# ziatdinovmax/pyroVED

Measured on AMD Instinct MI355X. Metric: images/sec (SVI step), higher is better.
Workload: dtype bf16; 1 GPU; C2 iVAE 28x28 invariances=['r','t'] latent_dim=2 bernoulli, batch 256 per GPU (global 256), bf16 MFMA operands for the hidden-layer contractions (fp32 accumulate; fp32 elsewhere); the guide (fc encoder, sample, split) runs in the decoder launch's prologue in fp32, SVI step = ELBO+grads+Adam; parallelism=dp1

## Files before the change

### pyroved_amd/csrc/pv_elementwise.hip

```cpp
#include "pv_common.h"
#include "pv_kernels.h"
#include "pv_wgrad_small.h"
#include "pv_side.h"
#include "pv_sdec_fused.h"


__device__ __forceinline__ float block_sum_256(float v, float* sm ) {
  v = pv_wave_sum(v);
  pv_lds_barrier();
  if ((threadIdx.x & 63) == 0) sm[threadIdx.x >> 6] = v;
  pv_lds_barrier();
  return (sm[0] + sm[1]) + (sm[2] + sm[3]);
}

__global__ __launch_bounds__(256) void pv_head_fwd_kernel(PvHead h) {
  __shared__ float sm[4];
  const int total = h.B * h.z_dim;
  float lp = 0.0f, lq = 0.0f;
  for (int e = threadIdx.x; e < total; e += 256) {
    const int b = e / h.z_dim, i = e % h.z_dim;
    const int ldh = h.ldh > 0 ? h.ldh : 2 * h.z_dim;
    const float mu = h.head[(int64_t)b * ldh + i];
    const float sp = h.head[(int64_t)b * ldh + h.z_dim + i];
    const float sig = h.scale_direct ? sp : pv_softplus(sp);
// ... 1032 lines not shown
  if (t < p.hb.z_dim)
    pv_head_bwd_elem(p.hb, b, t, [&](int c) { return sh_tp[c]; }, [&](int k) { return sh_dzc[k]; },
                     p.enc_n > 0 ? sh_dh : nullptr);
  if (p.K > 0 && t == 0) {
    const float b1 = p.beta_disc, lK = logf((float)K);
    const float* al = p.alpha + (int64_t)b * K;
    float dot = 0.0f;
    for (int k = 0; k < K; ++k) {
      const float da = -(sh_ll[k] - b1 * lK - b1 * logf(al[k]) - b1);
      dot += al[k] * da;
    }
    const int ldh = p.hb.ldh > 0 ? p.hb.ldh : 2 * p.hb.z_dim;
    for (int k = 0; k < K; ++k) {
      const float da = -(sh_ll[k] - b1 * lK - b1 * logf(al[k]) - b1);
      p.hb.dhead[(int64_t)b * ldh + 2 * p.hb.z_dim + k] = al[k] * (da - dot);
      if (p.enc_n > 0) sh_dh[2 * p.hb.z_dim + k] = al[k] * (da - dot);
    }
  }
  LB_STAMP(4);
  if (p.enc_n <= 0) return;
  pv_lds_barrier();
  const int ne = p.enc_n;
  int cur = 0;
  {
    const pv_layer hd = p.enc_head, ll_ = p.enc_l[ne - 1];
    const float* Wh = p.enc_params + hd.w_off;
    for (int k = t; k < ll_.out_dim; k += 256) {
      float v = 0.0f;
      if (chain && k == t) {
#pragma unroll
        for (int o = 0; o < 16; ++o) v += o < hd.out_dim ? sh_dh[o] * whd[o] : 0.0f;
        for (int o = 16; o < hd.out_dim; ++o) v += sh_dh[o] * Wh[(int64_t)o * hd.in_dim + k];
      } else {
        for (int o = 0; o < hd.out_dim; ++o) v += sh_dh[o] * Wh[(int64_t)o * hd.in_dim + k];
      }
      v *= pv_act_grad2((chain && k == t) ? pf_act1 : p.enc_act[ne - 1][(int64_t)b * ll_.out_dim + k], 0.0f, ll_.act);
      p.enc_dp[ne - 1][(int64_t)b * ll_.out_dim + k] = v;
      sh_e[cur][k] = v;
    }
    pv_lds_barrier();
  }
  LB_STAMP(5);
  for (int li = ne - 1; li > 0; --li) {
    const pv_layer l = p.enc_l[li], lp = p.enc_l[li - 1];
    const float* W = p.enc_params + l.w_off;
    const bool pre = li == ne - 1;
    const int k = ck, half = chalf;
    const int jh = l.out_dim >> 1, j0 = half * jh;
    float v = 0.0f;
    if (k < l.in_dim) {
      if (!pre) {
        const float* wc = W + k;
#pragma unroll
        for (int u = 0; u < 16; ++u)
#pragma unroll
          for (int i = 0; i < 4; ++i) wv4[u][i] = (4 * u + i < jh) ? wc[(int64_t)(j0 + 4 * u + i) * l.in_dim] : 0.0f;
      }
      f32x4 acc4 = {0.0f, 0.0f, 0.0f, 0.0f};
#pragma unroll
      for (int u = 0; u < 16; ++u)
        if (4 * u < jh) acc4 += *reinterpret_cast<const f32x4*>(&sh_e[cur][j0 + 4 * u]) * wv4[u];
      v = (acc4[0] + acc4[1]) + (acc4[2] + acc4[3]);
    }
    sh_p[half][k] = v;
    pv_lds_barrier();
    if (half == 0 && k < l.in_dim) {
      float y = sh_p[0][k] + sh_p[1][k];
      const float hv = pre ? pf_act0 : p.enc_act[li - 1][(int64_t)b * lp.out_dim + k];
      y *= pv_act_grad2(hv, 0.0f, lp.act);
      p.enc_dp[li - 1][(int64_t)b * lp.out_dim + k] = y;
      sh_e[cur ^ 1][k] = y;
    }
    pv_lds_barrier();
    cur ^= 1;
  }
  LB_STAMP(6);
}

__global__ __launch_bounds__(256) void pv_latent_bwd_kernel(PvLatentBwd p) { pv_latent_bwd_block(p, blockIdx.x); }

__global__ __launch_bounds__(256) void pv_latent_bwd_reduce_kernel(PvLatentBwd p, const float* __restrict__ part,
                                                                   int G_, float* __restrict__ Gr, PvFusedOffsets o,
                                                                   int cd, int fmt) {
  __shared__ f32x4 smr[4][64];
#ifndef LB_EXP
#define LB_EXP 0
#endif
  const int nred = pv_fused_reduce_blocks(fmt);
  if ((int)blockIdx.x < nred) { if (!(LB_EXP & 1)) pv_sdec_fused_reduce_block(part, G_, Gr, o, cd, 0, blockIdx.x, smr, fmt); }
  else if (!(LB_EXP & 2)) pv_latent_bwd_block(p, blockIdx.x - nred);
}

int pv_latent_bwd_reduce(const PvLatentBwd& p, const float* part, int grid, float* G, const PvFusedOffsets& o, int cd,
                         hipStream_t s, int fmt) {
  if (p.H > 512 || p.lat_in > 64 + (p.K > 0 ? p.K : 0) || p.hb.z_dim > 256 || p.K > 128) return PV_EINVAL;
  PV_LAUNCH_FORK(pv_latent_bwd_reduce_kernel, dim3(pv_fused_reduce_blocks(fmt) + p.hb.B), dim3(256), 0, s, p, part, grid, G, o, cd, fmt);
  PV_LAUNCH_CHECK();
  return 0;
}

__global__ __launch_bounds__(256) void pv_rec_wgrad_kernel(const float* __restrict__ part, int G_, float* __restrict__ Gr, PvFusedOffsets o,
                                                           int cd, int fmt, PvWgradSmall w, PvRecAdam ra, int rwx) {
  __shared__ f32x4 smr[4][64];
  __shared__ float wpart[WG_WAVES][16][17];
  __shared__ float wrpart[WG_WAVES][16];
  const int nred = pv_fused_reduce_blocks(fmt), id = (int)blockIdx.x;
  if (id < nred) { if (!(rwx & 1)) pv_sdec_fused_reduce_block(part, G_, Gr, o, cd, 0, id, smr, fmt, (rwx & 4) ? PvRecAdam{} : ra); return; }
  if (rwx & 2) return;
  pv_wgrad_small_block(w, id - nred, (int)gridDim.x - nred, wpart, wrpart);
}

int pv_rec_wgrad(const float* part, int grid, float* G, const PvFusedOffsets& o, int cd, int fmt, const PvGemm* gs, int n,
                 const PvAdamFuse* adam, const PvFinishArgs* fin, hipStream_t s, unsigned* tick) {
  PvWgradSmall w;
  int guests = 0;
  const int tiles = pv_wgrad_small_fill(w, gs, n, adam, fin, &guests);
  if (tiles < 0) return tiles;
  const int fin_blocks = (fin && fin->scalars) ? 1 : 0;
  if (tick && !fin_blocks) return PV_EINVAL;
  w.tick = tick;
  PvRecAdam ra{};
  if (adam) { ra.a = *adam; ra.on = 1; }
  static const int rwx = pv_exp_int("PV_RW_EXP", 0);
  hipLaunchKernelGGL(pv_rec_wgrad_kernel, dim3(pv_fused_reduce_blocks(fmt) + tiles + fin_blocks), dim3(256), 0, s, part, grid, G, o, cd,
                     fmt, w, ra, rwx);
  PV_LAUNCH_CHECK();
  return 0;
}

int pv_latent_bwd(const PvLatentBwd& p, hipStream_t s) {
  if (p.H > 512 || p.lat_in > 64 + (p.K > 0 ? p.K : 0) || p.hb.z_dim > 256 || p.K > 128) return PV_EINVAL;
  hipLaunchKernelGGL(pv_latent_bwd_kernel, dim3(p.hb.B), dim3(256), 0, s, p);
  PV_LAUNCH_CHECK();
  return 0;
}

__global__ void pv_adam_kernel(float* __restrict__ p, float* __restrict__ g, float* __restrict__ m,
                               float* __restrict__ v, int64_t n, float b1, float b2, float eps, float step_size,
                               float bc2_sqrt) {
  for (int64_t i = (int64_t)blockIdx.x * blockDim.x + threadIdx.x; i < n; i += (int64_t)gridDim.x * blockDim.x) {
    pv_adam_update(p, g, m, v, i, g[i], b1, b2, eps, step_size, bc2_sqrt);
  }
}

__global__ void pv_adam_hist_kernel(float* __restrict__ p, float* __restrict__ g, float* __restrict__ m,
                                    float* __restrict__ v, int64_t n, float b1, float b2, float eps, float step_size,
                                    float bc2_sqrt, const float* __restrict__ ssrc, float* __restrict__ sdst, int ns) {
  if (blockIdx.x == 0 && (int)threadIdx.x < ns) sdst[threadIdx.x] = ssrc[threadIdx.x];
  for (int64_t i = (int64_t)blockIdx.x * blockDim.x + threadIdx.x; i < n; i += (int64_t)gridDim.x * blockDim.x) {
    pv_adam_update(p, g, m, v, i, g[i], b1, b2, eps, step_size, bc2_sqrt);
  }
}

extern "C" int pv_adam_step_hist(float* params, float* grads, float* m, float* v, int64_t n, float lr, float beta1,
                                 float beta2, float eps, int32_t step, const float* scalars_src, float* scalars_dst,
                                 int32_t n_scalars, void* stream) {
  PV_RANGE("pv_adam_step_hist");
  if (step < 1 || n < 0 || n_scalars < 0 || n_scalars > 256 || (n_scalars > 0 && (!scalars_src || !scalars_dst)))
    return PV_EINVAL;
  const double bc1 = 1.0 - pow((double)beta1, (double)step);
  const double bc2 = 1.0 - pow((double)beta2, (double)step);
  int blocks = (int)((n + 255) / 256);
  if (blocks > 2048) blocks = 2048;
  if (blocks < 1) blocks = 1;
  hipLaunchKernelGGL(pv_adam_hist_kernel, dim3(blocks), dim3(256), 0, (hipStream_t)stream, params, grads, m, v, n, beta1,
                     beta2, eps, (float)((double)lr / bc1), (float)sqrt(bc2), scalars_src, scalars_dst, (int)n_scalars);
  PV_LAUNCH_CHECK();
  return 0;
}

extern "C" int pv_adam_step(float* params, float* grads, float* m, float* v, int64_t n, float lr, float beta1,
                            float beta2, float eps, int32_t step, void* stream) {
  PV_RANGE("pv_adam_step");
  if (n <= 0) return 0;
  if (step < 1) return PV_EINVAL;
  const double bc1 = 1.0 - pow((double)beta1, (double)step);
  const double bc2 = 1.0 - pow((double)beta2, (double)step);
  const float step_size = (float)((double)lr / bc1);
  const float bc2_sqrt = (float)sqrt(bc2);
  int blocks = (int)((n + 255) / 256);
  if (blocks > 2048) blocks = 2048;
  hipLaunchKernelGGL(pv_adam_kernel, dim3(blocks), dim3(256), 0, (hipStream_t)stream, params, grads, m, v, n, beta1,
                     beta2, eps, step_size, bc2_sqrt);
  PV_LAUNCH_CHECK();
  return 0;
}

__global__ void pv_lik_elem_kernel(const float* __restrict__ a, const float* __restrict__ x, int64_t M, int lik,
                                   int sigmoid_out, float sig, float* __restrict__ loc, float* __restrict__ llrow,
                                   float* __restrict__ dlda, const float* __restrict__ pw, int64_t per) {
  for (int64_t e = (int64_t)blockIdx.x * blockDim.x + threadIdx.x; e < M; e += (int64_t)gridDim.x * blockDim.x) {
    float ll, d, lv;
    pv_lik_one(a[e], x[e], lik, sigmoid_out, sig, ll, d, lv);
    if (pw) { const float w = pw[e % per]; ll *= w; d *= w; }
    if (loc) loc[e] = lv;
    if (llrow) llrow[e] = ll;
    if (dlda) dlda[e] = d;
  }
}

__global__ __launch_bounds__(256) void pv_lik_rows_kernel(const float* __restrict__ a, const float* __restrict__ x, int64_t per,
                                                          int lik, int sigmoid_out, float sig, float* __restrict__ loc,
                                                          float* __restrict__ dlda, float* __restrict__ llb,
                                                          const float* __restrict__ pw) {
  __shared__ float sm[4];
  const int64_t base = (int64_t)blockIdx.x * per;
// ... 134 lines not shown
```

### pyroved_amd/csrc/pv_particles.hip

```cpp
#include "pv_particles.h"
#include <cmath>

#define PX_THREADS 128
#define PX_MAX_Z 256
#define PX_MAX_LAT 256

template <class D> __device__ __forceinline__ int px_coord_cols(const D& d) {
  if (d.coord_dim == 1) return d.has_t ? 1 : 0;
  if (d.coord_dim == 2) return (d.has_r ? 1 : 0) + (d.has_t ? 2 : 0) + (d.has_s ? 1 : 0);
  return 0;
}

__global__ __launch_bounds__(PX_THREADS) void pv_particle_expand_kernel(PvParticleExpand e) {
  __shared__ float sm[16];
  __shared__ float sh_z[PX_MAX_Z];
  __shared__ float sh_in[PX_MAX_LAT];
  const int b = blockIdx.x, t = threadIdx.x, zd = e.z_dim;
  const int idx = px_coord_cols(e), L = zd - idx, lat_in = L + e.c_dim;
  const float inv_p = 1.0f / (float)e.P;
  float lp = 0.0f, lq = 0.0f;
  for (int p = 0; p < e.P; ++p) {
    const int64_t s = (int64_t)p * e.B + b;
    for (int i = t; i < zd; i += PX_THREADS) {
      const float mu = e.head[(int64_t)b * e.ldh + i];
// ... 100 lines not shown
        for (int n = t; n < p.N; n += 256) {
          a[0] += p.llrow[r0 + n];
          if (!p.fwd_only)
            for (int c = 0; c < 4; ++c) a[1 + c] += p.rowtp[(int64_t)c * p.M + r0 + n];
        }
        for (int c = 0; c < 5; ++c) {
          const float v = pv_block_sum(a[c], sm);
          if (t == 0) sh_a[c] = v;
        }
      }
      if (!p.fwd_only) {
        for (int j = t; j < p.H; j += 256) {
          const float* ph = p.part_hz + (s * p.kmax) * p.H + j;
          float v = 0.0f;
          for (int kk = 0; kk < p.kmax; ++kk) v += ph[(int64_t)kk * p.H];
          p.dhz[s * p.H + j] = v;
          sh_dhz[j] = v;
        }
        __syncthreads();
        if (t < n_content) {
          float v = 0.0f;
          for (int j = 0; j < p.H; ++j) v += sh_dhz[j] * p.Wz[(int64_t)j * p.lat_in + t];
          sh_dzc[t] = v;
        }
      }
    }
    __syncthreads();
    const float w = p.sw[s];
    if (t == 0) ll_acc += w * (p.ll_s ? p.ll_s[s] : sh_a[0]);
    if (!p.fwd_only && t < zd) {
      const float dz = pv_head_dz(p.hb, t, [&](int c) { return sh_a[1 + c]; }, [&](int k) { return sh_dzc[k]; });
      const int64_t e = s * zd + t;
      float g, ds;
      pv_head_bwd_math_kl(p.hb.kl_mode, dz, p.hb.z[e], p.hb.head[(int64_t)b * ldh + t], p.hb.z_scale[(int64_t)b * zd + t], p.hb.eps[e],
                          p.hb.head[(int64_t)b * ldh + zd + t], p.hb.beta * w, p.hb.scale_direct, g, ds);
      acc_g += g;
      acc_ds += ds;
    }
    __syncthreads();
  }
  if (t == 0) p.llb[b] = p.llb_add ? ll_acc + p.llb_add[b] : ll_acc;
  if (p.fwd_only) return;
  if (t < zd) {
    p.hb.dhead[(int64_t)b * ldh + t] = acc_g;
    p.hb.dhead[(int64_t)b * ldh + zd + t] = acc_ds;
    sh_dh[t] = acc_g;
    sh_dh[zd + t] = acc_ds;
  }
  if (p.enc_n <= 0) return;
  __syncthreads();
  const int ne = p.enc_n;
  int cur = 0;
  {
    const pv_layer hd = p.enc_head, l = p.enc_l[ne - 1];
    const float* Wh = p.enc_params + hd.w_off;
    for (int k = t; k < l.out_dim; k += 256) {
      float v = 0.0f;
      for (int o = 0; o < hd.out_dim; ++o) v += sh_dh[o] * Wh[(int64_t)o * hd.in_dim + k];
      v *= pv_act_grad2(p.enc_act[ne - 1][(int64_t)b * l.out_dim + k], 0.0f, l.act);
      p.enc_dp[ne - 1][(int64_t)b * l.out_dim + k] = v;
      sh_e[cur][k] = v;
    }
    __syncthreads();
  }
  for (int li = ne - 1; li > 0; --li) {
    const pv_layer l = p.enc_l[li], lp = p.enc_l[li - 1];
    const float* W = p.enc_params + l.w_off;
    for (int k = t; k < l.in_dim; k += 256) {
      float v = 0.0f;
      for (int j = 0; j < l.out_dim; ++j) v += sh_e[cur][j] * W[(int64_t)j * l.in_dim + k];
      v *= pv_act_grad2(p.enc_act[li - 1][(int64_t)b * lp.out_dim + k], 0.0f, lp.act);
      p.enc_dp[li - 1][(int64_t)b * lp.out_dim + k] = v;
      sh_e[cur ^ 1][k] = v;
    }
    __syncthreads();
    cur ^= 1;
  }
}

__global__ __launch_bounds__(256) void pv_particle_bwd_kernel(PvParticleBwd p) { pv_particle_bwd_block(p, blockIdx.x); }

__global__ __launch_bounds__(256) void pv_particle_bwd_reduce_kernel(PvParticleBwd p, const float* __restrict__ part, int G_,
                                                                     float* __restrict__ Gr, PvFusedOffsets o, int cd, int fmt) {
  __shared__ f32x4 smr[4][64];
  const int nred = pv_fused_reduce_blocks(fmt);
  if ((int)blockIdx.x < nred) pv_sdec_fused_reduce_block(part, G_, Gr, o, cd, 0, blockIdx.x, smr, fmt);
  else pv_particle_bwd_block(p, blockIdx.x - nred);
}

static int particle_bwd_check(const PvParticleBwd& p) {
  if (p.P < 1 || p.hb.B < 1 || p.hb.z_dim < 1 || p.hb.z_dim > PX_MAX_Z || !p.sw || !p.llb) return PV_EINVAL;
  if (p.llkb) {
    if (!p.fwd_only && (!p.dzc || (p.hb.coord_dim > 0 && !p.dtp))) return PV_EINVAL;
  } else {
    if (p.H > 512 || p.lat_in > PX_MAX_LAT || p.kmax < 1) return PV_EINVAL;
    if (!p.part_rs && !p.llrow) return PV_EINVAL;
    if (!p.fwd_only && (!p.part_hz || !p.dhz || !p.Wz || (!p.part_rs && !p.rowtp))) return PV_EINVAL;
  }
  if (p.enc_n > 0) {
    if (p.enc_head.out_dim != 2 * p.hb.z_dim) return PV_EINVAL;
    for (int i = 0; i < p.enc_n; ++i)
      if (p.enc_l[i].out_dim > 256) return PV_EINVAL;
  }
  return 0;
}

int pv_particle_bwd(const PvParticleBwd& p, hipStream_t s) {
  PV_TRY(particle_bwd_check(p));
  hipLaunchKernelGGL(pv_particle_bwd_kernel, dim3(p.hb.B), dim3(256), 0, s, p);
  PV_LAUNCH_CHECK();
  return 0;
}

int pv_particle_bwd_reduce(const PvParticleBwd& p, const float* part, int grid, float* G, const PvFusedOffsets& o, int cd,
                           hipStream_t s, int rec_fmt) {
  PV_TRY(particle_bwd_check(p));
  hipLaunchKernelGGL(pv_particle_bwd_reduce_kernel, dim3(pv_fused_reduce_blocks(rec_fmt) + p.hb.B), dim3(256), 0, s, p, part, grid, G, o,
                     cd, rec_fmt);
  PV_LAUNCH_CHECK();
  return 0;
}

__global__ __launch_bounds__(64) void pv_renyi_weights_kernel(PvRenyiWeights r) {
  __shared__ float sh_a[PV_RENYI_MAX_P], sh_lp[PV_RENYI_MAX_P], sh_lq[PV_RENYI_MAX_P];
  const int b = blockIdx.x, t = threadIdx.x, zd = r.z_dim;
  const float oma = 1.0f - r.alpha;
  for (int p = 0; p < r.P; ++p) {
    const int64_t s = (int64_t)p * r.B + b;
    float lp = 0.0f, lq = 0.0f;
    for (int i = t; i < zd; i += 64) {
      const float z = r.z[s * zd + i], e = r.eps[s * zd + i], sig = r.z_scale[(int64_t)b * zd + i];
      lq += -(e * e) / 2.0f - logf(sig) - LOG_SQRT_2PI;
      lp += -(z * z) / 2.0f - LOG_SQRT_2PI;
    }
    lp = r.beta * pv_wave_sum(lp);
    lq = r.beta * pv_wave_sum(lq);
    if (t == 0) {
      sh_lp[p] = lp;
      sh_lq[p] = lq;
      sh_a[p] = oma * (r.llkb[s] + (lp - lq));
    }
  }
  if (t != 0) return;
  float m = sh_a[0];
  for (int p = 1; p < r.P; ++p) m = fmaxf(m, sh_a[p]);
  float sum = 0.0f;
  for (int p = 0; p < r.P; ++p) sum += expf(sh_a[p] - m);
  const float inv = 1.0f / sum, lsum = logf(sum);
  float klp = 0.0f, klq = 0.0f, ent = 0.0f;
  for (int p = 0; p < r.P; ++p) {
    const int64_t s = (int64_t)p * r.B + b;
    const float d = sh_a[p] - m, w = expf(d) * inv;
    r.sw[s] = w;
    if (r.weights_out) r.weights_out[s] = w;
    klp += w * sh_lp[p];
    klq += w * sh_lq[p];
    ent -= w * (d - lsum);
  }
  r.kl_part[2 * b] = klp;
  r.kl_part[2 * b + 1] = klq;
  r.c[b] = (ent - logf((float)r.P)) / oma;
}

int pv_renyi_weights(const PvRenyiWeights& r, hipStream_t s) {
  if (r.B < 1 || r.P < 1 || r.P > PV_RENYI_MAX_P || r.z_dim < 1 || !std::isfinite(r.alpha) || r.alpha == 1.0f) return PV_EINVAL;
  if (!r.llkb || !r.z || !r.eps || !r.z_scale || !r.sw || !r.kl_part || !r.c) return PV_EINVAL;
  hipLaunchKernelGGL(pv_renyi_weights_kernel, dim3(r.B), dim3(64), 0, s, r);
// ... 4 lines not shown
```

### pyroved_amd/csrc/pv_sdec_fused.h

```cpp
#pragma once
#include "pv_common.h"

#define FD_H 128
#define FD_UNIT 16
#define FD_WAVES 8
#define FD_REC (2 * FD_H * FD_H + 14 * FD_H)
#define PV_RS_W 8
#define FB_WIMG_BYTES (4 * FD_H * FD_H * 2 + 256)

struct PvFused {
  const float* x;
  const float* grid;
  const float* tp;
  const float* hz;
  float hz_scale;
  const float *Wc, *bc;
  const float *W1, *b1;
  const float *W2, *b2;
  const float *wo, *bo;
  float* llrow;
  float* loc;
  float* rowtp;
  float* part_hz;
  float* part_rs;
// ... 24 lines not shown
  pv_layer enc0, enc1, head;
  const float* x; int64_t ldx;
  const float* eps;
  float* eact0; float* eact1;
  float* head_out;
  float* z; float* z_scale; float* z_loc_out; float* z_scale_out;
  float* tp;
  float* kl_part;
  float* hz; const float* Wz;
  int lat_in, z_dim, coord_dim, has_r, has_t, has_s;
  float tp0, tp1, sc_prior, beta;
  int img_per_wg;
#define PV_CHAIN_GENERIC_LOOP 2
  int chain;
  float* dhead; int ldh;
  float* edp0; float* edp1;
  float* llb;
  int coop;
  unsigned* coop_flags;
};
#if defined(__HIP_DEVICE_COMPILE__)
typedef const __attribute__((address_space(4))) PvEncFold* PvEncFoldArg;
__device__ __forceinline__ PvEncFoldArg pv_kernarg_fold() {
  const __attribute__((address_space(4))) char* k = (const __attribute__((address_space(4))) char*)__builtin_amdgcn_kernarg_segment_ptr();
  PvEncFoldArg p = (PvEncFoldArg)(k + ((sizeof(PvFused) + alignof(PvEncFold) - 1) / alignof(PvEncFold)) * alignof(PvEncFold));
  asm volatile("" : "+s"(p));
  return p;
}
#else
typedef const PvEncFold* PvEncFoldArg;
__device__ inline PvEncFoldArg pv_kernarg_fold() { return nullptr; }
#endif
#define PV_GUIDE_IMG_MAX_BATCH 384
struct PvFbPrep;
bool pv_guide_img_ok(const PvEncFold& e, int B);
int pv_guide_img_launch(const PvEncFold& e, const PvFbPrep* prep, float hz_mul, int B, hipStream_t s, int kl_mode = PV_KL_SAMPLED);
bool pv_sdec_fused_w8_fold_ok(const PvFused& f, int grid);
bool pv_sdec_fused_fold_ok(const PvFused& f, int grid, bool x3);

bool pv_sdec_fused_supported(const pv_ivae_plan* p);
int pv_sdec_fused_grid(int64_t units);
int pv_sdec_fused_kmax(int n_pix, int64_t units, int grid);
int pv_sdec_fused_launch(const PvFused& f, int grid, bool grads, hipStream_t s);
bool pv_sdec_fused_trunk_supported(const pv_ivae_plan* p);
bool pv_sdec_fused_mc_supported(const pv_ivae_plan* p);
int pv_sdec_fused_mc_launch(const PvFused& f, int C, int grid, bool grads, hipStream_t s, bool weighted = false);
bool pv_sdec_fused_mc_weighted_supported(const pv_ivae_plan* p);
int pv_sdec_fused_mc_reduce_out(const float* part, int grid, float* G, int64_t wo_off, int64_t bo_off, int C, hipStream_t s);
int pv_sdec_fused_bf16_prep(const PvFused& f, bool grads, bool x3, hipStream_t s);
struct PvFbPrep;
PvFbPrep pv_sdec_fused_bf16_prep_args(const PvFused& f, bool grads, bool x3);
bool pv_sdec_fused_w8_qswap();
int pv_sdec_fused_bf16_launch(const PvFused& f, int grid, bool grads, bool x3, hipStream_t s, const PvEncFold* fold = nullptr,
                              const PvEncFold* chain = nullptr);
int pv_sdec_fused_w8_launch(const PvFused& f, int grid, bool grads, hipStream_t s, const PvEncFold* fold = nullptr);
int pv_sdec_fused_w8x3_launch(const PvFused& f, int grid, bool grads, hipStream_t s, int waves);
int64_t pv_sdec_fused_w8x3_park_bytes(int grid);
int pv_sdec_fused_w8h_launch(const PvFused& f, int grid, bool ds, hipStream_t s);
int64_t pv_sdec_fused_bf16_park_bytes(bool x3, int64_t units, int grid, int sel);
int pv_sdec_fused_bf16_waves(bool x3, int64_t units, int sel);
int pv_sdec_fused_bf16_record_fmt(bool x3, int64_t units, int sel);
bool pv_sdec_fused_sel_valid(int fused, int sel);
struct PvFusedOffsets { int64_t W1, b1, W2, b2, Wc, wo, bo; };
int pv_sdec_fused_reduce(const float* part, int grid, float* G, const PvFusedOffsets& o, int cd, int dwo_slots,
                         hipStream_t s);

#define PV_FUSED_REDUCE_BLOCKS (((2 * FD_H * FD_H + 5 * FD_H + 1 + 3) / 4 + 63) / 64)
#define PV_REC_ROWMAJOR 0
#define PV_REC_LANE_F32 1
#define PV_REC_LANE_BF16 2
#define PV_FUSED_REDUCE_VEC_BLOCKS (((5 * FD_H + 1 + 3) / 4 + 63) / 64)
#define PV_FUSED_REDUCE_MAT_BLOCKS_F32 ((2 * FD_H * FD_H / 4) / 64)
#define PV_FUSED_REDUCE_MAT_BLOCKS_BF16 ((2 * (FD_H / 2) * FD_H / 4) / 64)
__host__ __device__ inline int pv_fused_reduce_mat_blocks(int fmt) {
  return fmt == PV_REC_LANE_BF16 ? PV_FUSED_REDUCE_MAT_BLOCKS_BF16 : PV_FUSED_REDUCE_MAT_BLOCKS_F32;
}
__host__ __device__ inline int pv_fused_reduce_blocks(int fmt) {
  return fmt == PV_REC_ROWMAJOR ? PV_FUSED_REDUCE_BLOCKS : pv_fused_reduce_mat_blocks(fmt) + PV_FUSED_REDUCE_VEC_BLOCKS;
}
#ifndef PV_RED_UNROLL
#define PV_RED_UNROLL 8
#endif
struct PvRecAdam { PvAdamFuse a; int on; };
__device__ __forceinline__ void pv_rec_out(float* __restrict__ Gr, int idx, float v, const PvRecAdam& ad) {
  if (ad.on) pv_adam_update(ad.a.p, ad.a.g, ad.a.m, ad.a.v, (Gr - ad.a.g) + idx, v, ad.a.b1, ad.a.b2, ad.a.eps, ad.a.step_size, ad.a.bc2_sqrt);
  else Gr[idx] = v;
}
template <int FMT>
__device__ __forceinline__ void pv_sdec_fused_reduce_block_lane(const float* __restrict__ part, int G_, float* __restrict__ Gr,
                                                                const PvFusedOffsets& o, int block, f32x4 (*sm)[64],
                                                                const PvRecAdam& ad = PvRecAdam{}) {
  const int c = threadIdx.x & 63, sl = threadIdx.x >> 6;
  const int per = (G_ + 3) / 4;
  const int w0 = sl * per, w1 = min(G_, w0 + per);
  const float* pbase = part + 4 * (block * 64 + c);
  f32x4 a = {0.0f, 0.0f, 0.0f, 0.0f}, b = {0.0f, 0.0f, 0.0f, 0.0f};
  if (FMT == PV_REC_LANE_BF16) {
    typedef unsigned int u32x4_ __attribute__((ext_vector_type(4)));
#pragma unroll PV_RED_UNROLL
    for (int w = w0; w < w1; ++w) {
      const u32x4_ v = *reinterpret_cast<const u32x4_*>(pbase + (int64_t)w * FD_REC);
      a[0] += __uint_as_float(v[0] << 16); a[1] += __uint_as_float(v[0] & 0xffff0000u);
      a[2] += __uint_as_float(v[1] << 16); a[3] += __uint_as_float(v[1] & 0xffff0000u);
      b[0] += __uint_as_float(v[2] << 16); b[1] += __uint_as_float(v[2] & 0xffff0000u);
      b[2] += __uint_as_float(v[3] << 16); b[3] += __uint_as_float(v[3] & 0xffff0000u);
    }
  } else {
#pragma unroll PV_RED_UNROLL
    for (int w = w0; w < w1; ++w) a += *reinterpret_cast<const f32x4*>(pbase + (int64_t)w * FD_REC);
  }
  sm[sl][c] = a;
  __syncthreads();
  const f32x4 ta = (sm[0][c] + sm[1][c]) + (sm[2][c] + sm[3][c]);
  f32x4 tb = b;
  if (FMT == PV_REC_LANE_BF16) {
    __syncthreads();
    sm[sl][c] = b;
    __syncthreads();
    tb = (sm[0][c] + sm[1][c]) + (sm[2][c] + sm[3][c]);
  }
  if (sl != 0) return;
  const int r = c & 15, q = c >> 4;
  if (FMT == PV_REC_LANE_BF16) {
    const int oo = block & 3, s_ = (block >> 2) & 1, wave = block >> 3, jp = wave >> 1, kh = wave & 1;
    const int row0 = 32 * jp + 16 * (s_ ^ kh) + 4 * q, col = 64 * kh + 16 * oo + r;
#pragma unroll
    for (int i = 0; i < 4; ++i) {
      pv_rec_out(Gr, o.W1 + (row0 + i) * FD_H + col, ta[i], ad);
      pv_rec_out(Gr, o.W2 + (row0 + i) * FD_H + col, tb[i], ad);
    }
  } else {
    const int kb = block & 7, s_ = (block >> 3) & 1, wave = (block >> 4) & 3, m = block >> 6;
    const int row0 = 16 * (2 * wave + s_) + 4 * q, col = 16 * kb + r;
    const int dst = m == 0 ? o.W1 : o.W2;
#pragma unroll
    for (int i = 0; i < 4; ++i) pv_rec_out(Gr, dst + (row0 + i) * FD_H + col, ta[i], ad);
  }
}
__device__ __forceinline__ void pv_sdec_fused_reduce_block(const float* __restrict__ part, int G_,
                                                           float* __restrict__ Gr, const PvFusedOffsets& o, int cd,
                                                           int dwo_slots, int block, f32x4 (*sm)[64], int fmt = PV_REC_ROWMAJOR,
                                                           const PvRecAdam& ad = PvRecAdam{}) {
  const int HH = FD_H * FD_H;
  const int total = 2 * HH + 5 * FD_H + 1;
  const int c = threadIdx.x & 63, sl = threadIdx.x >> 6;
  if (fmt != PV_REC_ROWMAJOR && block < pv_fused_reduce_mat_blocks(fmt)) {
    if (fmt == PV_REC_LANE_BF16) pv_sdec_fused_reduce_block_lane<PV_REC_LANE_BF16>(part, G_, Gr, o, block, sm, ad);
    else pv_sdec_fused_reduce_block_lane<PV_REC_LANE_F32>(part, G_, Gr, o, block, sm, ad);
    return;
  }
  const int e = fmt != PV_REC_ROWMAJOR ? 2 * HH + ((block - pv_fused_reduce_mat_blocks(fmt)) * 64 + c) * 4 : (block * 64 + c) * 4;
  const int per = (G_ + 3) / 4;
  const int w0 = sl * per, w1 = min(G_, w0 + per);
  f32x4 v = {0.0f, 0.0f, 0.0f, 0.0f};
  if (e < total) {
    const bool slots = dwo_slots && e >= 2 * HH + 4 * FD_H && e < 2 * HH + 5 * FD_H;
    if (slots) {
      for (int w = w0; w < w1; ++w) {
        const float* p8 = part + (int64_t)w * FD_REC + 2 * HH + 6 * FD_H + (e - (2 * HH + 4 * FD_H));
        f32x4 a = {0.0f, 0.0f, 0.0f, 0.0f};
        for (int k = 0; k < FD_WAVES; ++k) a += *reinterpret_cast<const f32x4*>(p8 + k * FD_H);
        v += a;
      }
    } else {
      const float* p = part + e;
#pragma unroll PV_RED_UNROLL
      for (int w = w0; w < w1; ++w) v += *reinterpret_cast<const f32x4*>(p + (int64_t)w * FD_REC);
    }
  }
  sm[sl][c] = v;
  __syncthreads();
  if (sl != 0 || e >= total) return;
  v = (sm[0][c] + sm[1][c]) + (sm[2][c] + sm[3][c]);
#pragma unroll
  for (int i = 0; i < 4; ++i) {
    const int ei = e + i;
    if (ei >= total) break;
    if (ei < HH) pv_rec_out(Gr, o.W1 + ei, v[i], ad);
    else if (ei < 2 * HH) pv_rec_out(Gr, o.W2 + (ei - HH), v[i], ad);
    else {
      const int k = ei - 2 * HH, seg = k / FD_H, j = k % FD_H;
      if (seg == 0) pv_rec_out(Gr, o.b1 + j, v[i], ad);
      else if (seg == 1) pv_rec_out(Gr, o.b2 + j, v[i], ad);
      else if (seg == 2) pv_rec_out(Gr, o.Wc + j * cd, v[i], ad);
      else if (seg == 3) { if (cd == 2) pv_rec_out(Gr, o.Wc + j * 2 + 1, v[i], ad); }
      else if (seg == 4) pv_rec_out(Gr, o.wo + j, v[i], ad);
      else pv_rec_out(Gr, o.bo, v[i], ad);
    }
  }
}
```

### pyroved_amd/csrc/pv_sdec_fused.hip

```cpp
#include "pv_sdec_fused_f32.h"
#include <stdlib.h>

template <bool GRADS>
__global__ __launch_bounds__(FD_THREADS, 2) void pv_sdec_fused_kernel(PvFused f) {
  extern __shared__ __attribute__((aligned(16))) float sm[];
  const int tid = threadIdx.x, wave = tid >> 6, lane = tid & 63, r = lane & 15, q = lane >> 4;
  const int g = blockIdx.x, G = gridDim.x;

  for (int idx = tid; idx < FD_H * (FD_H / 4); idx += FD_THREADS) {
    const int row = idx >> 5, c4 = idx & 31;
    *reinterpret_cast<f32x4*>(sm + OFF_W1 + row * LDW + 4 * c4) = reinterpret_cast<const f32x4*>(f.W1)[idx];
    *reinterpret_cast<f32x4*>(sm + OFF_W2 + row * LDW + 4 * c4) = reinterpret_cast<const f32x4*>(f.W2)[idx];
  }
  for (int j = tid; j < FD_H; j += FD_THREADS) {
    sm[OFF_WC0 + j] = f.Wc[j * f.cd];
    sm[OFF_WC1 + j] = f.cd == 2 ? f.Wc[j * 2 + 1] : 0.0f;
    sm[OFF_BC + j] = f.bc[j];
    sm[OFF_WO + j] = f.wo[j];
    sm[OFF_B1 + j] = f.b1[j];
    sm[OFF_B2 + j] = f.b2[j];
  }
  for (int j = tid; j < FD_WAVES * FD_H; j += FD_THREADS) sm[OFF_DWO + j] = 0.0f;
  __syncthreads();

// ... 139 lines not shown
      if (wave == c) { fd_stage_write(stA, tA, r, q); fd_stage_write(stB, tB, r, q); }
      __syncthreads();
      fd_wgrad_consume(stA, stB, accW1, db1, wave, r, q);
      __syncthreads();
    }
    if (active) {
      float d0 = 0.0f, d1 = 0.0f;
#pragma unroll
      for (int jb = 0; jb < 8; ++jb) {
        const f32x4 w0 = *reinterpret_cast<const f32x4*>(sm + OFF_WC0 + 16 * jb + 4 * q);
        const f32x4 w1 = *reinterpret_cast<const f32x4*>(sm + OFF_WC1 + 16 * jb + 4 * q);
#pragma unroll
        for (int i = 0; i < 4; ++i) { d0 += tC[jb][i] * w0[i]; d1 += tC[jb][i] * w1[i]; }
      }
      d0 = fd_sum_q(d0);
      d1 = fd_sum_q(d1);
      if (q == 0) {
        f.rowtp[row] = sc * (d1 * u0c - d0 * u1c);
        f.rowtp[f.M + row] = d0 * u0c + d1 * u1c;
        f.rowtp[2 * f.M + row] = d0;
        f.rowtp[3 * f.M + row] = d1;
      }
    }
    for (int c = 0; c < ((f.ablate & 2) ? 0 : nact); ++c) {
      if (wave == c) {
        fd_stage_write(stA, tC, r, q);
        if (q == 0) { sm[OFF_INFO + r] = x0; sm[OFF_INFO + 16 + r] = x1; }
        if (lane == 0) reinterpret_cast<int*>(sm + OFF_INFO)[32] = b;
      }
      __syncthreads();
      const int bc = reinterpret_cast<const int*>(sm + OFF_INFO)[32];
      if (bc != cur_b) {
        if (cur_b >= 0) flush_hz(cur_b);
        cur_b = bc;
        ahz = 0.0f;
      }
#pragma unroll
      for (int s = 0; s < 4; ++s) {
        const float v = stA[(4 * s + q) * LDST + 16 * wave + r];
        ahz += v;
        aWc0 += v * sm[OFF_INFO + 4 * s + q];
        aWc1 += v * sm[OFF_INFO + 16 + 4 * s + q];
      }
      __syncthreads();
    }
  }
  if (!GRADS) return;

  if (cur_b >= 0) flush_hz(cur_b);
  float* rec = f.part + (int64_t)g * FD_REC;
#pragma unroll
  for (int kb = 0; kb < 8; ++kb)
#pragma unroll
    for (int i = 0; i < 4; ++i) {
      rec[(16 * wave + 4 * q + i) * FD_H + 16 * kb + r] = accW1[kb][i];
      rec[FD_H * FD_H + (16 * wave + 4 * q + i) * FD_H + 16 * kb + r] = accW2[kb][i];
    }
  const float t1 = fd_sum_q(db1), t2 = fd_sum_q(db2), tc0 = fd_sum_q(aWc0), tc1 = fd_sum_q(aWc1);
  if (q == 0) {
    rec[2 * FD_H * FD_H + 16 * wave + r] = t1;
    rec[2 * FD_H * FD_H + FD_H + 16 * wave + r] = t2;
    rec[2 * FD_H * FD_H + 2 * FD_H + 16 * wave + r] = tc0;
    rec[2 * FD_H * FD_H + 3 * FD_H + 16 * wave + r] = tc1;
  }
  const float tb = pv_wave_sum(dbo);
  if (lane == 0) sm[OFF_RED + wave] = tb;
  __syncthreads();
  if (tid < FD_H) {
    float v = 0.0f;
#pragma unroll
    for (int w = 0; w < FD_WAVES; ++w) v += sm[OFF_DWO + w * FD_H + tid];
    rec[2 * FD_H * FD_H + 4 * FD_H + tid] = v;
  }
  if (tid == 0) {
    float v = 0.0f;
    for (int w = 0; w < FD_WAVES; ++w) v += sm[OFF_RED + w];
    rec[2 * FD_H * FD_H + 5 * FD_H] = v;
  }
}

__global__ __launch_bounds__(256) void pv_sdec_fused_reduce_kernel(const float* __restrict__ part, int G_,
                                                                   float* __restrict__ Gr, PvFusedOffsets o, int cd,
                                                                   int dwo_slots) {
  __shared__ f32x4 sm[4][64];
  pv_sdec_fused_reduce_block(part, G_, Gr, o, cd, dwo_slots, blockIdx.x, sm);
}

int pv_sdec_fused_reduce(const float* part, int grid, float* G, const PvFusedOffsets& o, int cd, int dwo_slots,
                         hipStream_t s) {
  hipLaunchKernelGGL(pv_sdec_fused_reduce_kernel, dim3(PV_FUSED_REDUCE_BLOCKS), dim3(256), 0, s, part, grid, G, o, cd,
                     dwo_slots);
  PV_LAUNCH_CHECK();
  return 0;
}

bool pv_sdec_fused_supported(const pv_ivae_plan* p) {
  return pv_sdec_fused_trunk_supported(p) && p->n_pix % FD_UNIT == 0 && p->out.out_dim == 1;
}

bool pv_sdec_fused_trunk_supported(const pv_ivae_plan* p) {
  if (!p || p->coord_dim < 1 || p->coord_dim > 2) return false;
  if (p->n_dec != 2) return false;
  const pv_layer& c = p->fc_coord;
  const pv_layer& l = p->fc_latent;
  if (c.out_dim != FD_H || c.b_off < 0 || l.out_dim != FD_H) return false;
  for (int i = 0; i < 2; ++i) {
    const pv_layer& d = p->dec[i];
    if (d.in_dim != FD_H || d.out_dim != FD_H || d.act != PV_ACT_TANH || d.b_off < 0) return false;
    if (d.w_off % 4 != 0) return false;
  }
  if (p->out.in_dim != FD_H || p->out.b_off < 0) return false;
  return true;
}

static int fd_num_cus() {
  static int cus = 0;
  if (cus == 0) {
    int dev = 0, n = 0;
    if (hipGetDevice(&dev) == hipSuccess &&
        hipDeviceGetAttribute(&n, hipDeviceAttributeMultiprocessorCount, dev) == hipSuccess && n > 0)
      cus = n;
    else
      cus = 256;
  }
  return cus;
}

int pv_sdec_fused_grid(int64_t units) {
  const int cus = fd_num_cus();
  return (int)(units < cus ? (units < 1 ? 1 : units) : cus);
}

int pv_sdec_fused_kmax(int n_pix, int64_t units, int grid) {
  const int64_t upb = n_pix / FD_UNIT;
  return (int)((upb * grid) / (units > 0 ? units : 1)) + 2;
}

int pv_sdec_fused_launch(const PvFused& f_in, int grid, bool grads, hipStream_t s) {
  PvFused f = f_in;
  static const int ablate = pv_exp_int("PV_FD_ABLATE", 0);
  f.ablate = ablate;
  const size_t lds = FD_LDS_FLOATS * sizeof(float);
  PV_TRY(pv_set_dynamic_lds(reinterpret_cast<const void*>(&pv_sdec_fused_kernel<true>), (int)lds));
  PV_TRY(pv_set_dynamic_lds(reinterpret_cast<const void*>(&pv_sdec_fused_kernel<false>), (int)lds));
  if (grads)
    hipLaunchKernelGGL(pv_sdec_fused_kernel<true>, dim3(grid), dim3(FD_THREADS), lds, s, f);
  else
    hipLaunchKernelGGL(pv_sdec_fused_kernel<false>, dim3(grid), dim3(FD_THREADS), lds, s, f);
  PV_LAUNCH_CHECK();
  return 0;
}
```

Before: 2.836 million images/s.

## Prefetch Adam state during gradient reduction and spread final sums across all waves

```diff
diff --git a/pyroved_amd/csrc/pv_elementwise.hip b/pyroved_amd/csrc/pv_elementwise.hip
--- a/pyroved_amd/csrc/pv_elementwise.hip
+++ b/pyroved_amd/csrc/pv_elementwise.hip
@@ -1138,7 +1138,7 @@
 __global__ __launch_bounds__(256) void pv_latent_bwd_reduce_kernel(PvLatentBwd p, const float* __restrict__ part,
                                                                    int G_, float* __restrict__ Gr, PvFusedOffsets o,
                                                                    int cd, int fmt) {
-  __shared__ f32x4 smr[4][64];
+  __shared__ PvRedLds smr;
 #ifndef LB_EXP
 #define LB_EXP 0
 #endif
@@ -1157,7 +1157,7 @@
 
 __global__ __launch_bounds__(256) void pv_rec_wgrad_kernel(const float* __restrict__ part, int G_, float* __restrict__ Gr, PvFusedOffsets o,
                                                            int cd, int fmt, PvWgradSmall w, PvRecAdam ra, int rwx) {
-  __shared__ f32x4 smr[4][64];
+  __shared__ PvRedLds smr;
   __shared__ float wpart[WG_WAVES][16][17];
   __shared__ float wrpart[WG_WAVES][16];
   const int nred = pv_fused_reduce_blocks(fmt), id = (int)blockIdx.x;
@@ -1165,6 +1165,9 @@
   if (rwx & 2) return;
   pv_wgrad_small_block(w, id - nred, (int)gridDim.x - nred, wpart, wrpart);
 }
+
+static uint64_t rec_wgrad_launches = 0;
+extern "C" uint64_t pv_debug_rec_wgrad_launches(void) { return __atomic_load_n(&rec_wgrad_launches, __ATOMIC_RELAXED); }
 
 int pv_rec_wgrad(const float* part, int grid, float* G, const PvFusedOffsets& o, int cd, int fmt, const PvGemm* gs, int n,
                  const PvAdamFuse* adam, const PvFinishArgs* fin, hipStream_t s, unsigned* tick) {
@@ -1178,6 +1181,7 @@
   PvRecAdam ra{};
   if (adam) { ra.a = *adam; ra.on = 1; }
   static const int rwx = pv_exp_int("PV_RW_EXP", 0);
+  __atomic_fetch_add(&rec_wgrad_launches, 1ull + ((uint64_t)ra.on << 32), __ATOMIC_RELAXED);
   hipLaunchKernelGGL(pv_rec_wgrad_kernel, dim3(pv_fused_reduce_blocks(fmt) + tiles + fin_blocks), dim3(256), 0, s, part, grid, G, o, cd,
                      fmt, w, ra, rwx);
   PV_LAUNCH_CHECK();
diff --git a/pyroved_amd/csrc/pv_particles.hip b/pyroved_amd/csrc/pv_particles.hip
--- a/pyroved_amd/csrc/pv_particles.hip
+++ b/pyroved_amd/csrc/pv_particles.hip
@@ -206,7 +206,7 @@
 
 __global__ __launch_bounds__(256) void pv_particle_bwd_reduce_kernel(PvParticleBwd p, const float* __restrict__ part, int G_,
                                                                      float* __restrict__ Gr, PvFusedOffsets o, int cd, int fmt) {
-  __shared__ f32x4 smr[4][64];
+  __shared__ PvRedLds smr;
   const int nred = pv_fused_reduce_blocks(fmt);
   if ((int)blockIdx.x < nred) pv_sdec_fused_reduce_block(part, G_, Gr, o, cd, 0, blockIdx.x, smr, fmt);
   else pv_particle_bwd_block(p, blockIdx.x - nred);
diff --git a/pyroved_amd/csrc/pv_sdec_fused.h b/pyroved_amd/csrc/pv_sdec_fused.h
--- a/pyroved_amd/csrc/pv_sdec_fused.h
+++ b/pyroved_amd/csrc/pv_sdec_fused.h
@@ -130,78 +130,127 @@
 #define PV_RED_UNROLL 8
 #endif
 struct PvRecAdam { PvAdamFuse a; int on; };
-__device__ __forceinline__ void pv_rec_out(float* __restrict__ Gr, int idx, float v, const PvRecAdam& ad) {
-  if (ad.on) pv_adam_update(ad.a.p, ad.a.g, ad.a.m, ad.a.v, (Gr - ad.a.g) + idx, v, ad.a.b1, ad.a.b2, ad.a.eps, ad.a.step_size, ad.a.bc2_sqrt);
+typedef f32x4 PvRedLds[2][4][64];
+struct PvRecOps { float p, m, v; };
+template <bool ADAM>
+__device__ __forceinline__ PvRecOps pv_rec_request(const float* __restrict__ Gr, int idx, const PvRecAdam& ad) {
+  PvRecOps q = {0.0f, 0.0f, 0.0f};
+  if (ADAM) { const int64_t i = (Gr - ad.a.g) + idx; q.p = ad.a.p[i]; q.m = ad.a.m[i]; q.v = ad.a.v[i]; }
+  return q;
+}
+__device__ __forceinline__ void pv_adam_update_ops(float* __restrict__ p, float* __restrict__ g, float* __restrict__ m,
+                                                   float* __restrict__ v, int64_t i, float gi, float pi, float mi, float vi,
+                                                   float b1, float b2, float eps, float step_size, float bc2_sqrt) {
+#pragma clang fp contract(off)
+  mi = mi + (gi - mi) * (1.0f - b1);
+  vi = vi * b2 + (1.0f - b2) * gi * gi;
+  const float denom = sqrtf(vi) / bc2_sqrt + eps;
+  p[i] = __builtin_fmaf(-step_size, mi / denom, pi);
+  m[i] = mi; v[i] = vi;
+  g[i] = 0.0f;
+}
+template <bool ADAM>
+__device__ __forceinline__ void pv_rec_fin(float* __restrict__ Gr, int idx, float v, const PvRecOps& q, const PvRecAdam& ad) {
+  if (ADAM) pv_adam_update_ops(ad.a.p, ad.a.g, ad.a.m, ad.a.v, (Gr - ad.a.g) + idx, v, q.p, q.m, q.v, ad.a.b1, ad.a.b2, ad.a.eps,
+                                ad.a.step_size, ad.a.bc2_sqrt);
   else Gr[idx] = v;
 }
-template <int FMT>
+template <typename V, typename Add, typename Req>
+__device__ __forceinline__ void pv_rec_stream(const float* __restrict__ p, int w0, int w1, Add add, Req request) {
+  const bool peel = w1 - w0 >= PV_RED_UNROLL;
+  const int wl = peel ? w1 - PV_RED_UNROLL : w1;
+#pragma unroll PV_RED_UNROLL
+  for (int w = w0; w < wl; ++w) add(*reinterpret_cast<const V*>(p + (int64_t)w * FD_REC));
+  V t[PV_RED_UNROLL];
+  if (peel) {
+#pragma unroll
+    for (int k = 0; k < PV_RED_UNROLL; ++k) t[k] = *reinterpret_cast<const V*>(p + (int64_t)(wl + k) * FD_REC);
+  }
+  request();
+  if (peel) {
+#pragma unroll
+    for (int k = 0; k < PV_RED_UNROLL; ++k) add(t[k]);
+  }
+}
+template <int FMT, bool ADAM>
 __device__ __forceinline__ void pv_sdec_fused_reduce_block_lane(const float* __restrict__ part, int G_, float* __restrict__ Gr,
-                                                                const PvFusedOffsets& o, int block, f32x4 (*sm)[64],
-                                                                const PvRecAdam& ad = PvRecAdam{}) {
+                                                                const PvFusedOffsets& o, int block, f32x4 (*sm)[4][64],
+                                                                const PvRecAdam& ad) {
   const int c = threadIdx.x & 63, sl = threadIdx.x >> 6;
   const int per = (G_ + 3) / 4;
   const int w0 = sl * per, w1 = min(G_, w0 + per);
   const float* pbase = part + 4 * (block * 64 + c);
+  float* lds = reinterpret_cast<float*>(sm);
+  const int r = c & 15, q = c >> 4;
+  int ia, ib = 0;
+  if (FMT == PV_REC_LANE_BF16) {
+    const int oo = block & 3, s_ = (block >> 2) & 1, wave = block >> 3, jp = wave >> 1, kh = wave & 1;
+    const int row0 = 32 * jp + 16 * (s_ ^ kh) + 4 * q, col = 64 * kh + 16 * oo + r;
+    ia = o.W1 + (row0 + sl) * FD_H + col;
+    ib = o.W2 + (row0 + sl) * FD_H + col;
+  } else {
+    const int kb = block & 7, s_ = (block >> 3) & 1, wave = (block >> 4) & 3, m = block >> 6;
+    const int row0 = 16 * (2 * wave + s_) + 4 * q, col = 16 * kb + r;
+    ia = (m == 0 ? o.W1 : o.W2) + (row0 + sl) * FD_H + col;
+  }
   f32x4 a = {0.0f, 0.0f, 0.0f, 0.0f}, b = {0.0f, 0.0f, 0.0f, 0.0f};
+  PvRecOps qa = {0.0f, 0.0f, 0.0f}, qb = {0.0f, 0.0f, 0.0f};
   if (FMT == PV_REC_LANE_BF16) {
     typedef unsigned int u32x4_ __attribute__((ext_vector_type(4)));
-#pragma unroll PV_RED_UNROLL
-    for (int w = w0; w < w1; ++w) {
-      const u32x4_ v = *reinterpret_cast<const u32x4_*>(pbase + (int64_t)w * FD_REC);
+    pv_rec_stream<u32x4_>(pbase, w0, w1, [&](const u32x4_ v) {
       a[0] += __uint_as_float(v[0] << 16); a[1] += __uint_as_float(v[0] & 0xffff0000u);
       a[2] += __uint_as_float(v[1] << 16); a[3] += __uint_as_float(v[1] & 0xffff0000u);
       b[0] += __uint_as_float(v[2] << 16); b[1] += __uint_as_float(v[2] & 0xffff0000u);
       b[2] += __uint_as_float(v[3] << 16); b[3] += __uint_as_float(v[3] & 0xffff0000u);
-    }
+    }, [&]() { qa = pv_rec_request<ADAM>(Gr, ia, ad); qb = pv_rec_request<ADAM>(Gr, ib, ad); });
   } else {
-#pragma unroll PV_RED_UNROLL
-    for (int w = w0; w < w1; ++w) a += *reinterpret_cast<const f32x4*>(pbase + (int64_t)w * FD_REC);
-  }
-  sm[sl][c] = a;
-  __syncthreads();
-  const f32x4 ta = (sm[0][c] + sm[1][c]) + (sm[2][c] + sm[3][c]);
-  f32x4 tb = b;
-  if (FMT == PV_REC_LANE_BF16) {
-    __syncthreads();
-    sm[sl][c] = b;
-    __syncthreads();
-    tb = (sm[0][c] + sm[1][c]) + (sm[2][c] + sm[3][c]);
-  }
-  if (sl != 0) return;
-  const int r = c & 15, q = c >> 4;
-  if (FMT == PV_REC_LANE_BF16) {
-    const int oo = block & 3, s_ = (block >> 2) & 1, wave = block >> 3, jp = wave >> 1, kh = wave & 1;
-    const int row0 = 32 * jp + 16 * (s_ ^ kh) + 4 * q, col = 64 * kh + 16 * oo + r;
+    pv_rec_stream<f32x4>(pbase, w0, w1, [&](const f32x4 v) { a += v; }, [&]() { qa = pv_rec_request<ADAM>(Gr, ia, ad); });
+  }
 #pragma unroll
-    for (int i = 0; i < 4; ++i) {
-      pv_rec_out(Gr, o.W1 + (row0 + i) * FD_H + col, ta[i], ad);
-      pv_rec_out(Gr, o.W2 + (row0 + i) * FD_H + col, tb[i], ad);
-    }
-  } else {
-    const int kb = block & 7, s_ = (block >> 3) & 1, wave = (block >> 4) & 3, m = block >> 6;
-    const int row0 = 16 * (2 * wave + s_) + 4 * q, col = 16 * kb + r;
-    const int dst = m == 0 ? o.W1 : o.W2;
-#pragma unroll
-    for (int i = 0; i < 4; ++i) pv_rec_out(Gr, dst + (row0 + i) * FD_H + col, ta[i], ad);
-  }
-}
-__device__ __forceinline__ void pv_sdec_fused_reduce_block(const float* __restrict__ part, int G_,
-                                                           float* __restrict__ Gr, const PvFusedOffsets& o, int cd,
-                                                           int dwo_slots, int block, f32x4 (*sm)[64], int fmt = PV_REC_ROWMAJOR,
-                                                           const PvRecAdam& ad = PvRecAdam{}) {
+  for (int i = 0; i < 4; ++i) {
+    lds[(sl * 4 + i) * 64 + c] = a[i];
+    if (FMT == PV_REC_LANE_BF16) lds[((4 + sl) * 4 + i) * 64 + c] = b[i];
+  }
+  pv_lds_barrier();
+  const float* la = lds + sl * 64 + c;
+  pv_rec_fin<ADAM>(Gr, ia, (la[0] + la[256]) + (la[512] + la[768]), qa, ad);
+  if (FMT == PV_REC_LANE_BF16) pv_rec_fin<ADAM>(Gr, ib, (la[1024] + la[1280]) + (la[1536] + la[1792]), qb, ad);
+}
+__device__ __forceinline__ int pv_rec_elem_index(int ei, const PvFusedOffsets& o, int cd) {
+  const int HH = FD_H * FD_H;
+  if (ei < HH) return o.W1 + ei;
+  if (ei < 2 * HH) return o.W2 + (ei - HH);
+  const int k = ei - 2 * HH, seg = k / FD_H, j = k % FD_H;
+  if (seg == 0) return o.b1 + j;
+  if (seg == 1) return o.b2 + j;
+  if (seg == 2) return o.Wc + j * cd;
+  if (seg == 3) return cd == 2 ? (int)(o.Wc + j * 2 + 1) : -1;
+  if (seg == 4) return o.wo + j;
+  return o.bo;
+}
+template <bool ADAM>
+__device__ __forceinline__ void pv_sdec_fused_reduce_block_on(const float* __restrict__ part, int G_,
+                                                              float* __restrict__ Gr, const PvFusedOffsets& o, int cd,
+                                                              int dwo_slots, int block, f32x4 (*sm)[4][64], int fmt,
+                                                              const PvRecAdam& ad) {
   const int HH = FD_H * FD_H;
   const int total = 2 * HH + 5 * FD_H + 1;
   const int c = threadIdx.x & 63, sl = threadIdx.x >> 6;
   if (fmt != PV_REC_ROWMAJOR && block < pv_fused_reduce_mat_blocks(fmt)) {
-    if (fmt == PV_REC_LANE_BF16) pv_sdec_fused_reduce_block_lane<PV_REC_LANE_BF16>(part, G_, Gr, o, block, sm, ad);
-    else pv_sdec_fused_reduce_block_lane<PV_REC_LANE_F32>(part, G_, Gr, o, block, sm, ad);
+    if (fmt == PV_REC_LANE_BF16) pv_sdec_fused_reduce_block_lane<PV_REC_LANE_BF16, ADAM>(part, G_, Gr, o, block, sm, ad);
+    else pv_sdec_fused_reduce_block_lane<PV_REC_LANE_F32, ADAM>(part, G_, Gr, o, block, sm, ad);
     return;
   }
-  const int e = fmt != PV_REC_ROWMAJOR ? 2 * HH + ((block - pv_fused_reduce_mat_blocks(fmt)) * 64 + c) * 4 : (block * 64 + c) * 4;
+  const int e0 = fmt != PV_REC_ROWMAJOR ? 2 * HH + (block - pv_fused_reduce_mat_blocks(fmt)) * 256 : block * 256;
+  const int e = e0 + 4 * c, ef = e0 + (int)threadIdx.x;
+  const int idx = ef < total ? pv_rec_elem_index(ef, o, cd) : -1;
   const int per = (G_ + 3) / 4;
   const int w0 = sl * per, w1 = min(G_, w0 + per);
   f32x4 v = {0.0f, 0.0f, 0.0f, 0.0f};
-  if (e < total) {
+  PvRecOps qf = {0.0f, 0.0f, 0.0f};
+  const auto request = [&]() { qf = pv_rec_request<ADAM>(Gr, max(idx, 0), ad); };
+  if (e >= total) request();
+  else {
     const bool slots = dwo_slots && e >= 2 * HH + 4 * FD_H && e < 2 * HH + 5 * FD_H;
     if (slots) {
       for (int w = w0; w < w1; ++w) {
@@ -210,30 +259,21 @@
         for (int k = 0; k < FD_WAVES; ++k) a += *reinterpret_cast<const f32x4*>(p8 + k * FD_H);
         v += a;
       }
+      request();
     } else {
-      const float* p = part + e;
-#pragma unroll PV_RED_UNROLL
-      for (int w = w0; w < w1; ++w) v += *reinterpret_cast<const f32x4*>(p + (int64_t)w * FD_REC);
+      pv_rec_stream<f32x4>(part + e, w0, w1, [&](const f32x4 x) { v += x; }, request);
     }
   }
-  sm[sl][c] = v;
-  __syncthreads();
-  if (sl != 0 || e >= total) return;
-  v = (sm[0][c] + sm[1][c]) + (sm[2][c] + sm[3][c]);
-#pragma unroll
-  for (int i = 0; i < 4; ++i) {
-    const int ei = e + i;
-    if (ei >= total) break;
-    if (ei < HH) pv_rec_out(Gr, o.W1 + ei, v[i], ad);
-    else if (ei < 2 * HH) pv_rec_out(Gr, o.W2 + (ei - HH), v[i], ad);
-    else {
-      const int k = ei - 2 * HH, seg = k / FD_H, j = k % FD_H;
-      if (seg == 0) pv_rec_out(Gr, o.b1 + j, v[i], ad);
-      else if (seg == 1) pv_rec_out(Gr, o.b2 + j, v[i], ad);
-      else if (seg == 2) pv_rec_out(Gr, o.Wc + j * cd, v[i], ad);
-      else if (seg == 3) { if (cd == 2) pv_rec_out(Gr, o.Wc + j * 2 + 1, v[i], ad); }
-      else if (seg == 4) pv_rec_out(Gr, o.wo + j, v[i], ad);
-      else pv_rec_out(Gr, o.bo, v[i], ad);
-    }
-  }
-}
+  sm[0][sl][c] = v;
+  pv_lds_barrier();
+  if (idx < 0) return;
+  const float* lf = reinterpret_cast<const float*>(sm) + threadIdx.x;
+  pv_rec_fin<ADAM>(Gr, idx, (lf[0] + lf[256]) + (lf[512] + lf[768]), qf, ad);
+}
+__device__ __forceinline__ void pv_sdec_fused_reduce_block(const float* __restrict__ part, int G_,
+                                                           float* __restrict__ Gr, const PvFusedOffsets& o, int cd,
+                                                           int dwo_slots, int block, f32x4 (*sm)[4][64], int fmt = PV_REC_ROWMAJOR,
+                                                           const PvRecAdam& ad = PvRecAdam{}) {
+  if (ad.on) pv_sdec_fused_reduce_block_on<true>(part, G_, Gr, o, cd, dwo_slots, block, sm, fmt, ad);
+  else pv_sdec_fused_reduce_block_on<false>(part, G_, Gr, o, cd, dwo_slots, block, sm, fmt, ad);
+}
diff --git a/pyroved_amd/csrc/pv_sdec_fused.hip b/pyroved_amd/csrc/pv_sdec_fused.hip
--- a/pyroved_amd/csrc/pv_sdec_fused.hip
+++ b/pyroved_amd/csrc/pv_sdec_fused.hip
@@ -245,7 +245,7 @@
 __global__ __launch_bounds__(256) void pv_sdec_fused_reduce_kernel(const float* __restrict__ part, int G_,
                                                                    float* __restrict__ Gr, PvFusedOffsets o, int cd,
                                                                    int dwo_slots) {
-  __shared__ f32x4 sm[4][64];
+  __shared__ PvRedLds sm;
   pv_sdec_fused_reduce_block(part, G_, Gr, o, cd, dwo_slots, blockIdx.x, sm);
 }
 
```

Result: faster. 2.941 million images/s (median of 6 runs) (+3.7%).
